# wonjune-kang/llm-speech-summarization

Measured on AMD Instinct MI355X. Metric: generated tokens/s of end-to-end generate_audio_response steps (encode + prefill + 256-token greedy decode), HuBERT-large -> Llama-3.2-3B; audio-sec/s reported beside it, encoder stage alone and in the pipeline, higher is better.
Workload: dtype bf16

## Files before the change

include/speechllm.h:

```cpp
#ifndef SPEECHLLM_H
#define SPEECHLLM_H

#include <stddef.h>
#include <stdint.h>

#ifdef __cplusplus
extern "C" {
#endif

typedef void* sl_stream;

enum sl_dtype { SL_F32 = 0, SL_BF16 = 1, SL_F16 = 2 };
enum sl_status {
  SL_OK = 0,
  SL_ERR_ARG = -1,
  SL_ERR_LAUNCH = -2,
  SL_ERR_UNSUPPORTED = -3
};
enum sl_act { SL_ACT_NONE = 0, SL_ACT_GELU = 1, SL_ACT_SILU_MUL = 2, SL_ACT_ROPE_KV = 3 };
enum sl_w_layout { SL_W_ROWMAJOR = 0, SL_W_PACKED = 1 };
#define SL_W_PACKED_E4M3 2
#define SL_W_PACKED_MXFP4 4

const char* sl_last_error(void);
// ... 22 lines not shown

size_t sl_w4_image_bytes(int32_t N, int32_t K);
int sl_pack_weight_mxfp4(const void* src, int64_t ld_src, void* dst, int32_t N, int32_t K, int32_t dtype, sl_stream stream);
int sl_pack_weight_mxfp4_host(const void* src, int64_t ld_src, void* dst, int32_t N, int32_t K, int32_t dtype);
int32_t sl_w4_max_rows(void);

size_t sl_mx_weight_image_bytes(int32_t N, int32_t K);
int sl_pack_weight_mx(const void* src, int64_t ld_src, void* dst, int32_t N, int32_t K, int32_t dtype, sl_stream stream);
int sl_pack_weight_mx_host(const void* src, int64_t ld_src, void* dst, int32_t N, int32_t K, int32_t dtype);
int sl_mxfp8_quantize_rows(const void* x, int64_t ldx, void* q, void* scales, int64_t M, int32_t K, int32_t dtype, sl_stream stream);
int sl_mxfp8_quantize_rows_host(const void* x, int64_t ldx, void* q, void* scales, int64_t M, int32_t K, int32_t dtype);
typedef struct {
  const void* Aq; int64_t lda; const void* a_scales;
  const void* W;
  void* C; int64_t ldc;
  const void* residual; int64_t ldr;
  int32_t M, N, K;
  int32_t dtype, act, out_f32;
} sl_gemm_mx_args;
int sl_gemm_mx(const sl_gemm_mx_args* a, sl_stream stream);

typedef struct {
  int32_t fuse_rms; float rms_eps;
  const float* rope_cos; const float* rope_sin;
  const int32_t* tok_pos; const int32_t* tok_seq;
  void* k_cache; void* v_cache;
  int32_t n_heads, n_kv_heads, max_ctx, reserved;
  void* split_ws; size_t split_ws_bytes;
  const float* rstd_in; float* rstd_out;
  void* norm_out; const void* norm_gain;
} sl_gemm_fused;
size_t sl_gemm_split_workspace_bytes(int32_t M, int32_t N, int32_t K, int32_t dtype);
int32_t sl_gemm_split_count(int32_t M, int32_t N, int32_t K, int32_t dtype);
int sl_gemm_fused_decode(const sl_gemm_args* a, const sl_gemm_fused* fx, sl_stream stream);

typedef struct {
  int32_t trans_a, trans_w, residual_f32, w_mod;
  void* aux_out;
  const int64_t* groups;
  int32_t groups_ext, reserved;
  float* amax_val; int32_t* amax_idx;
  const float* ln_mr; const float* ln_u; const float* ln_c; float* stats_out;
  void* sk_ws; size_t sk_ws_bytes;
  int32_t post_op, post_reserved;
  float drop_p; float post_reserved_f;
  uint64_t drop_seed;
  int64_t drop_ld;
  const void* post_in; int64_t post_ld;
  float* colsum_out;
  int32_t* deferred_splits;
} sl_gemm_ex_args;
enum { SL_POST_NONE = 0, SL_POST_DROPOUT = 1, SL_POST_GELU_BWD = 2, SL_POST_SILU_MUL_BWD = 3 };
int sl_gemm_ex(const sl_gemm_args* a, const sl_gemm_ex_args* ex, sl_stream stream);
size_t sl_gemm_streamk_workspace_bytes(void);
int32_t sl_gemm_ln_fold_ok(int32_t M, int32_t N, int32_t K, int32_t dtype);
int sl_layernorm_fold_build(const void* W, const void* gain, const void* beta, const void* bias, void* Wf, float* u, float* c, int32_t N,
                            int32_t K, int32_t dtype, sl_stream stream);
int sl_layernorm_stats_finalize(const float* stats, int32_t segs, int64_t rows, int32_t cols, float eps, float* mr, sl_stream stream);
int sl_layernorm_stats(const void* x, int64_t rows, int32_t cols, float eps, float* mr, int32_t dtype, sl_stream stream);

int sl_layernorm(const void* x, void* y, const void* gamma, const void* beta, int64_t rows, int32_t cols,
                 float eps, int32_t gelu, int32_t dtype, sl_stream stream);

int sl_rmsnorm(const void* x, void* y, const void* w, int64_t rows, int32_t cols, float eps, int32_t dtype,
               sl_stream stream);

// ... 516 lines not shown
```

llm-speech-summarization_amd/_lib.py:

```python
from __future__ import annotations

import ctypes as C
import os
from dataclasses import dataclass, field

import torch

_HERE = os.path.dirname(os.path.abspath(__file__))
LIB_PATH = (os.environ.get("SL_LIB_PATH") if os.environ.get("SL_DEV") == "1" else None) or os.path.join(_HERE, "libspeechllm.so")

SL_F32, SL_BF16, SL_F16 = 0, 1, 2
KV_MODEL_DTYPE, KV_FP8_E4M3 = 0, 1
ACT_NONE, ACT_GELU, ACT_SILU_MUL, ACT_ROPE_KV = 0, 1, 2, 3
POST_NONE, POST_DROPOUT, POST_GELU_BWD, POST_SILU_MUL_BWD = 0, 1, 2, 3
W_ROWMAJOR, W_PACKED, W_PACKED_E4M3 = 0, 1, 2
W_PACKED_MXFP4 = 4
WDEC_MODEL_DTYPE, WDEC_E4M3 = 0, 1
WDEC_MXFP4 = 4
WDEC_MX_LINEAR = 5
COMM_ID_BYTES = 128
MAX_DECODE_BATCH = 2048

c_i32, c_i64, c_f32, c_vp, c_sz = C.c_int32, C.c_int64, C.c_float, C.c_void_p, C.c_size_t

# ... 219 lines not shown
    "sl_tuning_reload": (c_i32, []),
    "sl_decode_graph_cache_clear": (c_i32, []),
    "sl_gemm": (c_i32, [C.POINTER(GemmArgs), c_vp]),
    "sl_gemm_streamk_workspace_bytes": (C.c_size_t, []),
    "sl_layernorm_fold_build": (c_i32, [c_vp, c_vp, c_vp, c_vp, c_vp, c_vp, c_vp, c_i32, c_i32, c_i32, c_vp]),
    "sl_weight_norm_bwd": (c_i32, [c_vp, c_vp, c_vp, c_vp, c_vp, c_vp, c_i32, c_i32, c_i32, c_vp]),
    "sl_weight_norm_bwd_workspace_bytes": (C.c_size_t, [c_i32]),
    "sl_comm_unique_id": (c_i32, [c_vp]),
    "sl_comm_init": (c_i32, [C.POINTER(c_vp), c_vp, c_i32, c_i32]),
    "sl_allreduce_sum": (c_i32, [c_vp, c_vp, c_i64, c_i32, c_vp]),
    "sl_comm_destroy": (c_i32, [c_vp]),
    "sl_comm_abort": (c_i32, [c_vp]),
    "sl_comm_rank": (c_i32, [c_vp]),
    "sl_comm_world": (c_i32, [c_vp]),
    "sl_pack_weight": (c_i32, [c_vp, c_i64, c_vp, c_i32, c_i32, c_i32, c_vp]),
    "sl_w8_image_bytes": (c_sz, [c_i32, c_i32]),
    "sl_pack_weight_e4m3": (c_i32, [c_vp, c_i64, c_vp, c_i32, c_i32, c_i32, c_vp]),
    "sl_pack_weight_e4m3_host": (c_i32, [c_vp, c_i64, c_vp, c_i32, c_i32, c_i32]),
    "sl_w8_max_rows": (c_i32, []),
    "sl_w4_image_bytes": (c_sz, [c_i32, c_i32]),
    "sl_pack_weight_mxfp4": (c_i32, [c_vp, c_i64, c_vp, c_i32, c_i32, c_i32, c_vp]),
    "sl_pack_weight_mxfp4_host": (c_i32, [c_vp, c_i64, c_vp, c_i32, c_i32, c_i32]),
    "sl_w4_max_rows": (c_i32, []),
    "sl_weight_format_info": (c_i32, [c_i32, C.POINTER(c_i32), C.POINTER(c_i32), C.POINTER(c_i32)]),
    "sl_mx_weight_image_bytes": (c_sz, [c_i32, c_i32]),
    "sl_pack_weight_mx": (c_i32, [c_vp, c_i64, c_vp, c_i32, c_i32, c_i32, c_vp]),
    "sl_pack_weight_mx_host": (c_i32, [c_vp, c_i64, c_vp, c_i32, c_i32, c_i32]),
    "sl_mxfp8_quantize_rows": (c_i32, [c_vp, c_i64, c_vp, c_vp, c_i64, c_i32, c_i32, c_vp]),
    "sl_mxfp8_quantize_rows_host": (c_i32, [c_vp, c_i64, c_vp, c_vp, c_i64, c_i32, c_i32]),
    "sl_gemm_mx": (c_i32, [C.POINTER(GemmMxArgs), c_vp]),
    "sl_gemm_fused_decode": (c_i32, [C.POINTER(GemmArgs), C.POINTER(GemmFused), c_vp]),
    "sl_gemm_split_workspace_bytes": (c_sz, [c_i32, c_i32, c_i32, c_i32]),
    "sl_gemm_split_count": (c_i32, [c_i32, c_i32, c_i32, c_i32]),
    "sl_attn_decode_workspace_bytes": (c_sz, [c_i32, c_i32, c_i32, c_i32]),
    "sl_attn_decode_split": (c_i32, [c_vp, c_i64, c_vp, c_vp, c_vp, c_vp, c_vp, c_i32, c_i32, c_i32, c_i32, c_i32, c_f32, c_i32, c_vp]),
    "sl_gemm_ex": (c_i32, [C.POINTER(GemmArgs), C.POINTER(GemmEx), c_vp]),
    "sl_gemm_ln_fold_ok": (c_i32, [c_i32, c_i32, c_i32, c_i32]),
    "sl_layernorm_stats_finalize": (c_i32, [c_vp, c_i32, c_i64, c_i32, c_f32, c_vp, c_vp]),
    "sl_layernorm_stats": (c_i32, [c_vp, c_i64, c_i32, c_f32, c_vp, c_i32, c_vp]),
    "sl_gelu_bwd": (c_i32, [c_vp, c_vp, c_vp, c_i64, c_i32, c_vp]),
    "sl_axpby": (c_i32, [c_vp, c_vp, c_f32, c_f32, c_i64, c_i32, c_vp]),
    "sl_adamw_blocks": (C.c_size_t, [c_i64]),
    "sl_adamw_step": (c_i32, [c_vp, c_vp, c_i32, c_i64, C.c_double, C.c_double, C.c_double, C.c_double, C.c_double, c_i64, c_vp]),
    "sl_attn_dropout_bwd": (c_i32, [c_vp, c_vp, c_vp, c_i64, c_i32, c_vp, c_i32, c_vp, c_i32, c_i32, c_i32, c_f32, C.c_uint64, c_i32, c_vp]),
    "sl_transpose_pad": (c_i32, [c_vp, c_i64, c_vp, c_i64, c_i32, c_i32, c_i32, c_i32, c_vp]),
    "sl_dropout": (c_i32, [c_vp, c_vp, c_vp, c_i64, c_f32, C.c_uint64, c_i32, c_vp]),
    "sl_silu_mul": (c_i32, [c_vp, c_vp, c_i64, c_i32, c_i32, c_vp]),
    "sl_silu_mul_bwd": (c_i32, [c_vp, c_vp, c_vp, c_i64, c_i32, c_i32, c_vp]),
    "sl_rope_inplace": (c_i32, [c_vp, c_vp, c_vp, c_vp, c_i64, c_i32, c_i32, c_i32, c_i32, c_i32, c_vp]),
    "sl_layernorm_bwd": (c_i32, [c_vp, c_vp, c_vp, c_vp, c_vp, c_vp, c_vp, c_i64, c_i32, c_f32, c_i32, c_i32, c_vp]),
    "sl_layernorm_bwd_ws_bytes": (c_sz, [c_i64, c_i32]),
    "sl_layernorm_bwd_ws": (c_i32, [c_vp, c_vp, c_vp, c_vp, c_vp, c_vp, c_vp, c_i64, c_i32, c_f32, c_i32, c_i32, c_vp, c_sz, c_vp]),
    "sl_rmsnorm_bwd": (c_i32, [c_vp, c_vp, c_vp, c_vp, c_i64, c_i32, c_f32, c_i32, c_vp]),
    "sl_colsum": (c_i32, [c_vp, c_i64, c_vp, c_i64, c_i32, c_i32, c_vp]),
    "sl_softmax_rows": (c_i32, [c_vp, c_vp, c_i64, c_i32, c_i32, c_i64, c_f32, c_i32, c_i32, c_vp]),
    "sl_softmax_bwd": (c_i32, [c_vp, c_vp, c_vp, c_i64, c_i32, c_i64, c_f32, c_i32, c_vp]),
    "sl_softmax_rows_var": (c_i32, [c_vp, c_vp, c_i64, c_i32, c_vp, c_i64, c_f32, c_i32, c_i32, c_vp]),
    "sl_softmax_bwd_var": (c_i32, [c_vp, c_vp, c_vp, c_i64, c_i32, c_vp, c_i64, c_f32, c_i32, c_vp]),
    "sl_ce_loss": (c_i32, [c_vp, c_vp, c_i64, c_i32, c_f32, c_vp, c_vp, c_i32, c_i32, c_vp]),
    "sl_soft_ce_loss": (c_i32, [c_vp, c_vp, c_i64, c_i32, c_f32, c_vp, c_vp, c_i32, c_i32, c_vp]),
    "sl_mse_loss": (c_i32, [c_vp, c_vp, c_i64, c_f32, c_vp, c_vp, c_i32, c_i32, c_vp]),
    "sl_kd_logit_losses": (c_i32, [c_vp, c_vp, c_vp, c_vp, c_vp, c_i64, c_i32, c_vp, c_i32, c_vp, c_i32, c_vp]),
    "sl_kd_mse_rows": (c_i32, [c_vp, c_vp, c_vp, c_vp, c_i64, c_i32, c_vp, c_i32, c_i32, c_vp, c_i32, c_vp]),
    "sl_avgpool_bwd": (c_i32, [c_vp, c_vp, c_i64, c_i32, c_i32, c_i32, c_i64, c_i32, c_vp]),
    "sl_col2im": (c_i32, [c_vp, c_vp, c_i64, c_i64, c_i32, c_i32, c_i32, c_i32, c_vp]),
    "sl_col2im_batch": (c_i32, [c_vp, c_vp, c_vp, c_i32, c_i64, c_i32, c_i32, c_i32, c_i32, c_vp]),
# ... 248 lines not shown
```

llm-speech-summarization_amd/csrc/api.hip:

```cpp
#include <stdarg.h>
#include <stdlib.h>

#include <atomic>
#include <mutex>

#include "common.h"

static thread_local char g_err[512] = "";

void sl_set_error(const char* fmt, ...) {
  va_list ap;
  va_start(ap, fmt);
  vsnprintf(g_err, sizeof(g_err), fmt, ap);
  va_end(ap);
}

extern "C" const char* sl_last_error(void) { return g_err; }

extern "C" int sl_version(void) { return SL_ABI_VERSION; }

extern "C" int sl_kv_quantize_e4m3_host(const float* x, uint8_t* out, int64_t n) {
  SL_CHECK_ARG(x != nullptr && out != nullptr && n >= 0, "sl_kv_quantize_e4m3_host: bad arguments");
  for (int64_t i = 0; i < n; ++i) out[i] = (uint8_t)sl_q8_e4m3(x[i]);
  return 0;
// ... 46 lines not shown
  e.t256_min_k = env_int("SL_T256_MIN_K", 1024);
  e.t256_phased = env_int("SL_T256_PHASED", 1);
  e.t256_by_rounds_pad = env_int("SL_T256_BY_ROUNDS_PAD", 1);
  e.decode_tiled = env_int("SL_DECODE_TILED", 1);
  e.stream_k = env_int("SL_STREAM_K", 1);
  e.split_k = env_int("SL_SPLIT_K", 1);
  e.wgrad_tr = env_int("SL_WGRAD_TR", 1);
  e.tt_max_splits = env_int("SL_TT_MAX_SPLITS", 8);
  e.lnbwd_nw = env_int("SL_LNBWD_NW", 16);
  e.skinny_alt = env_int("SL_SKINNY_ALT", 0);
  e.prefill_share_prefix = env_int("SL_PREFILL_SHARE_PREFIX", 1);
  e.prefill_prune_last = env_int("SL_PREFILL_PRUNE_LAST", 1);
  e.gemm_ko = env_int("SL_GEMM_KO", 0);
  { const char* sp = getenv("SL_GEMM_STAMP_PTR"); e.gemm_stamp_ptr = (sp && sp[0]) ? strtoull(sp, nullptr, 16) : 0ull; }
  const char* g = getenv("SL_DISABLE_GLDS");
  e.disable_glds = (g && g[0] == '1') ? 1 : ((g && g[0] == '2') ? 2 : 0);
  e.direct_epilogue = env_int("SL_DIRECT_EPILOGUE", 0);
  e.gemm_gm = env_int("SL_GEMM_GM", 8);
  e.attn_full_min = env_int("SL_ATTN_FULL_MIN", 32);
  e.attn_force_split = getenv("SL_ATTN_FORCE_SPLIT") != nullptr;
  { const int ks = env_int("SL_ATTN_DECODE_KS", 128); e.attn_decode_ks = (ks == 64 || ks == 65) ? ks : 128; }
  e.attn_split_merge = env_int("SL_ATTN_SPLIT_MERGE", -1);
  e.attn_generic = env_int("SL_ATTN_GENERIC", 0);
  e.attn_qt = env_int("SL_ATTN_QT", 0);
  e.norm_single_row = env_int("SL_NORM_SINGLE_ROW", 0);
  e.no_ln_fold = env_int("SL_NO_LN_FOLD", 0);
  e.no_swap_epilogue = env_int("SL_NO_SWAP_EPILOGUE", 0);
  e.gemm_log = env_int("SL_GEMM_LOG", 0);
  e.no_wgrad_stream = env_int("SL_NO_WGRAD_STREAM", 0);
  e.stream_splits = e.stream_nwv = e.stream_mt = 0;
  e.stream_nl = env_int("SL_STREAM_NL", 0);
  e.stream_wide = env_int("SL_STREAM_WIDE", 1);
  e.stream_wsplits = env_int("SL_STREAM_WSPLITS", 0);
  e.stream_fixup = env_int("SL_STREAM_FIXUP", 0);
  const char* sc = getenv("SL_STREAM_CFG");
  if (sc && sc[0]) {
    int sp = 0, nwv = 0, mt = 0;
    const int n = sscanf(sc, "%d,%d,%d", &sp, &nwv, &mt);
    if (n >= 2) {
      if (sp >= 1 && sp <= 64) e.stream_splits = sp;
      if (nwv == 2 || nwv == 4) e.stream_nwv = nwv;
    }
    if (n == 3 && (mt == 8 || mt == 16)) e.stream_mt = mt;
  }
  return &e;
}

const SlEnv& sl_env() {
  const SlEnv* e = g_env.load(std::memory_order_acquire);
  if (!e) {
    std::lock_guard<std::mutex> lk(g_env_mu);
    e = g_env.load(std::memory_order_relaxed);
    if (!e) {
      e = env_load();
      g_env.store(e, std::memory_order_release);
    }
  }
  return *e;
}

static thread_local int g_family_rows = 0;
int sl_family_rows(int rows) { return g_family_rows > rows ? g_family_rows : rows; }
int sl_family_pin(int rows) {
  const int prev = g_family_rows;
  g_family_rows = rows > 0 ? rows : 0;
  return prev;
}
// ... 7 lines not shown
```

llm-speech-summarization_amd/csrc/gemm.hip:

```cpp
#include <stdlib.h>

#include "common.h"
#include "gemm_internal.h"
#include "wformat.h"

#include "gemm_epilogue.h"

template <typename T, int ACT>
__global__ __launch_bounds__(256, 2) void gemm_tiled_kernel(GemmP p) {
  constexpr int VEC = Vec16<T>::VEC;
  constexpr int BK = TROWB / (int)sizeof(T);
  __shared__ __attribute__((aligned(16))) unsigned char smem[2][2][TBM * TROWB];

  const int tid = threadIdx.x, lane = tid & 63, wave = tid >> 6;
  const int wm = wave >> 1, wn = wave & 1;
  const int r = lane & 15, q = lane >> 4;

  int bm, bn;
  tile_patch_coords(xcd_remap(blockIdx.x, p.tiles_m * p.tiles_n), p.tiles_m, p.tiles_n, 8, bm, bn);
  const int z = blockIdx.y;

  int64_t a_off; int wz;
  if (!resolve_group(p, z, bm, a_off, wz)) return;
  const T* A = (const T*)p.A + a_off;
// ... 1155 lines not shown
  const size_t sk_ws_bytes = ex ? ex->sk_ws_bytes : 0;
  SL_CHECK_ARG(!sk_ws || ((uintptr_t)sk_ws & 15) == 0, "sl_gemm_ex: sk_ws must be 16-byte aligned");
  if (a->dtype == SL_F32) return gemm_typed<float>(a, p, sx, st, sk_ws, sk_ws_bytes, e);
  if (a->dtype == SL_F16) return gemm_typed<f16_t>(a, p, sx, st, sk_ws, sk_ws_bytes, e);
  return gemm_typed<bf16_t>(a, p, sx, st, sk_ws, sk_ws_bytes, e);
}

int sl_gemm_impl(const sl_gemm_args* a, const sl_gemm_fused* fx, const sl_gemm_ex_args* ex, hipStream_t st) { return gemm_impl(a, fx, ex, st, nullptr); }

int sl_gemm_top1_lse_impl(const sl_gemm_args* a, const sl_gemm_ex_args* ex, float* amax_sum, hipStream_t st) {
  SL_CHECK_ARG(ex != nullptr && amax_sum != nullptr, "sl_gemm_top1_lse: null ex args or amax_sum");
  return gemm_impl(a, nullptr, ex, st, amax_sum);
}

extern "C" int sl_gemm_top1_lse(const sl_gemm_args* a, const sl_gemm_ex_args* ex, float* amax_sum, sl_stream stream) {
  return sl_gemm_top1_lse_impl(a, ex, amax_sum, (hipStream_t)stream);
}

int sl_gemm_top1_lse_tgt_impl(const sl_gemm_args* a, const sl_gemm_ex_args* ex, float* amax_sum, const int32_t* tgt_col, float* tgt_val, hipStream_t st) {
  SL_CHECK_ARG(ex != nullptr && amax_sum != nullptr, "sl_gemm_top1_lse_tgt: null ex args or amax_sum");
  return gemm_impl(a, nullptr, ex, st, amax_sum, tgt_col, tgt_val);
}

extern "C" int sl_gemm_top1_lse_tgt(const sl_gemm_args* a, const sl_gemm_ex_args* ex, float* amax_sum, const int32_t* tgt_col, float* tgt_val, sl_stream stream) {
  return sl_gemm_top1_lse_tgt_impl(a, ex, amax_sum, tgt_col, tgt_val, (hipStream_t)stream);
}

extern "C" int32_t sl_gemm_split_count(int32_t M, int32_t N, int32_t K, int32_t dtype) {
  M = sl_family_rows(M);
  if (M <= sl_env().stream_min_m || M <= 0 || N <= 0 || K <= 0 || K % (dtype == SL_F32 ? 32 : 64) != 0) return 1;
  return sl_gemm_stream_splits(M, N, K, dtype);
}

extern "C" size_t sl_gemm_split_workspace_bytes(int32_t M, int32_t N, int32_t K, int32_t dtype) {
  if (sl_family_rows(M) <= sl_env().stream_min_m || M <= 0 || N <= 0 || K <= 0) return 0;
  return sl_gemm_stream_ws_bytes(M, N, K, dtype);
}

extern "C" int32_t sl_gemm_ln_fold_ok(int32_t M, int32_t N, int32_t K, int32_t dtype) { return sl_gemm_rows_epilogue_ok(M, N, K, dtype) ? 1 : 0; }

extern "C" int sl_gemm(const sl_gemm_args* a, sl_stream stream) { return sl_gemm_impl(a, nullptr, nullptr, (hipStream_t)stream); }

extern "C" int sl_gemm_ex(const sl_gemm_args* a, const sl_gemm_ex_args* ex, sl_stream stream) {
  SL_CHECK_ARG(ex != nullptr, "sl_gemm_ex: null ex args");
  return sl_gemm_impl(a, nullptr, ex, (hipStream_t)stream);
}

extern "C" int sl_gemm_fused_decode(const sl_gemm_args* a, const sl_gemm_fused* fx, sl_stream stream) {
  SL_CHECK_ARG(fx != nullptr, "sl_gemm_fused_decode: null fused args");
  return sl_gemm_impl(a, fx, nullptr, (hipStream_t)stream);
}
```

llm-speech-summarization_amd/csrc/gemm_internal.h:

```cpp
#pragma once
#include "common.h"

struct GemmP {
  const void* A; int64_t lda, sA;
  const void* W; int64_t ldw, sW;
  void* C; int64_t ldc, sC;
  const void* bias; int64_t sBias;
  const void* res; int64_t ldr, sR;
  int M, N, K, out_f32;
  int tiles_m, tiles_n;
  int ta, tw;
  void* aux;
  int res_f32;
  const int64_t* grp;
  int w_mod;
  int64_t cx, rx, wx;
  int grp_ext;
  int grp_kslab;
  int gm;
  int direct_epi;
  const float* ln_mr;
  const float* ln_u;
  const float* ln_c;
  float* stats_out;
// ... 109 lines not shown
int sl_gemm128_ring_launch(const GemmP& p, int stages, dim3 grid, hipStream_t st);
enum : int { SL_TT_TWO_STAGE = 0, SL_TT_RING = 1, SL_TT_BATCHED = 2 };
int sl_gemm_tt_kernel_launch(const GemmP& p, int form, dim3 grid, int slabs_per_run, hipStream_t st);

bool sl_gemm_post_ok(int64_t M, int N, int K, int dtype);
bool sl_gemm_rows_epilogue_ok(int M, int N, int K, int dtype);

struct SkinnyX {
  const float* cos; const float* sin;
  const int32_t* pos; const int32_t* seq;
  void* kc; void* vc;
  int nh, nkv, max_ctx, fuse_rms;
  float eps;
  int kv8;
  const float* rstd_in;
  float* rstd_out;
  void* norm_out;
  const void* norm_gain;
};
constexpr int SL_ACT_ROPE_KV8 = 64 + SL_ACT_ROPE_KV;
constexpr bool sl_act_is_rope_kv(int act) { return act == SL_ACT_ROPE_KV || act == SL_ACT_ROPE_KV8; }
template <typename T>
__device__ __forceinline__ void kv_store(void* cache, int64_t at, float v, int kv8) {
  const T t = from_f32<T>(v);
  if constexpr (sizeof(T) == 2) {
    if (kv8) { ((uint8_t*)cache)[at] = (uint8_t)sl_q8_e4m3(to_f32(t)); return; }
  }
  ((T*)cache)[at] = t;
}

int sl_gemm_stream_launch(GemmP& p, const SkinnyX& sx, int dtype, int act, void* split_ws, size_t split_ws_bytes, hipStream_t st);
size_t sl_gemm_stream_ws_bytes(int M, int N, int K, int dtype);
int sl_gemm_stream_splits(int M, int N, int K, int dtype);
```

llm-speech-summarization_amd/csrc/gemm_stream.hip:

```cpp
#include <type_traits>
#include <stdlib.h>

#include <atomic>

#include "gemm_internal.h"

struct StreamX {
  float* part;
  float* part_ss;
  int splits, sps;
  int np;
  int* cnt;
  float* ss_part;
};

__device__ __forceinline__ void st_sc1_16(float* ptr, const f32x4& v) {
  asm volatile("global_store_dwordx4 %0, %1, off sc1" ::"v"(ptr), "v"(v) : "memory");
}
__device__ __forceinline__ void ld_sc1_16(f32x4& v, const float* ptr) {
  asm volatile("global_load_dwordx4 %0, %1, off sc1" : "=v"(v) : "v"(ptr) : "memory");
}
__device__ __forceinline__ void vm_drain16(f32x4 (&v)[16]) {
  asm volatile("s_waitcnt vmcnt(0)"
               : "+v"(v[0]), "+v"(v[1]), "+v"(v[2]), "+v"(v[3]), "+v"(v[4]), "+v"(v[5]), "+v"(v[6]), "+v"(v[7]), "+v"(v[8]), "+v"(v[9]), "+v"(v[10]),
                 "+v"(v[11]), "+v"(v[12]), "+v"(v[13]), "+v"(v[14]), "+v"(v[15])
               :
               : "memory");
}

template <typename T, int ACT>
__device__ __forceinline__ void stream_epilogue4(const GemmP& p, const SkinnyX& sx, int m, int gf, int n4, const float (&a)[4], const float (&b)[4]) {
  const T* bias = (const T*)p.bias;
  if constexpr (ACT == SL_ACT_SILU_MUL) {
    const int ocol = (gf >> 1) * 16 + n4;
    if (ocol >= (p.N >> 1)) return;
#pragma unroll
    for (int i = 0; i < 4; ++i) {
      float g = a[i], u = b[i];
      if (bias) { g += to_f32(bias[gf * 16 + n4 + i]); u += to_f32(bias[(gf + 1) * 16 + n4 + i]); }
      store_out<T>(p, p.C, p.res, m, ocol + i, silu(g) * u);
    }
  } else if constexpr (ACT == SL_ACT_ROPE_KV) {
    if (gf * 16 >= p.N) return;
    const int hh = gf >> 3, j = (gf & 7) >> 1;
    const int pos = sx.pos[m];
    if (hh < sx.nh + sx.nkv) {
// ... 257 lines not shown
    for (int d = 0; d < D - 1; ++d)
      if (n_full + d < n_it) stage(d, n_full + d);
    if constexpr (FUSE) {
#pragma unroll
      for (int j = 0; j < NSS; ++j) {
        const int t = j * NWV + wn;
        if (t < MT && (r >> 2) == q) ssl[t * 16 + r] = ssacc[j][r & 3];
      }
    }
  }
  __syncthreads();
  if (wave >= NWV) return;

  float ssum[MT];
#pragma unroll
  for (int t = 0; t < MT; ++t) {
    ssum[t] = 0.f;
    if (fuse) ssum[t] = ssl[t * 16 + r];
  }
  stream_finish<T, MT, ACT, RF>(p, sx, s, acc, ssum, fuse, m0, sp, fi0, nfrag, nb == 0 && wn == 0, q, r);
}

template <typename T, int ACT>
__global__ __launch_bounds__(768) void gemm_stream_wide_kernel(GemmP p, SkinnyX sx, StreamX s) {
  constexpr int VEC = Vec16<T>::VEC;
  constexpr int KSTEP = MMA<T>::KSTEP;
  constexpr int CW = 8;
  constexpr int MTW = 4, RFW = 4;
  constexpr int BM = 256, BF = 8;
  constexpr int SLAB_X = BM * TROWB, SLAB_W = BF * 2 * 1024, SLOT = SLAB_X + SLAB_W;
  constexpr int NSLOT = 3;
  constexpr int NDMA = 12;
  extern __shared__ __attribute__((aligned(16))) unsigned char smem[];
  __shared__ int fx_last[2];
  __shared__ float fx_ss[4][2][64];

  const int tid = threadIdx.x, lane = tid & 63;
  const int wave = __builtin_amdgcn_readfirstlane(tid >> 6);
  const int r = lane & 15, q = lane >> 4;
  const int mblocks = (p.M + BM - 1) / BM;
  const int nfrag = (p.N + 15) >> 4;
  const int xj = blockIdx.x >> 3, nb = (xj / mblocks) * 8 + (blockIdx.x & 7);
  if (nb * BF >= nfrag) return;
  const int mblock = xj % mblocks;
  const int m0 = mblock * BM;
  const int sp = blockIdx.z;
  const int nks = p.K / KSTEP;
  const int g_lo = sp * s.sps;
  const int g_hi = min(nks >> 1, g_lo + s.sps);
  const int n_it = g_hi - g_lo;
  const int g_last = g_hi - 1;
  const int wm = (wave >> 1) & 3, wn = wave & 1;
  const int mw = m0 + wm * 64, fi0 = nb * BF + wn * RFW;

  f32x4 acc[RFW][MTW];
  float ssum[MTW];
#pragma unroll
  for (int t = 0; t < MTW; ++t) {
    ssum[t] = 0.f;
#pragma unroll
    for (int f = 0; f < RFW; ++f) acc[f][t] = f32x4{0.f, 0.f, 0.f, 0.f};
  }

  if (wave >= CW) {
    const int lw = wave - CW;
    const T* A = (const T*)p.A;
    const T* W = (const T*)p.W;
    const int ch = (lane & 7) ^ ((lane >> 3) & 7);
// ... 56 lines not shown
      }
    };
    __builtin_amdgcn_s_barrier();
    rd(0, 0, 0);
    for (int it = 0; it < n_it; ++it) {
      __builtin_amdgcn_sched_barrier(0);
      rd(it, 1, 1);
      mma(0);
      __builtin_amdgcn_sched_barrier(0);
      asm volatile("s_waitcnt lgkmcnt(0)" ::: "memory");
      __builtin_amdgcn_s_barrier();
      rd(it + 1, 0, 0);
      mma(1);
      __builtin_amdgcn_sched_barrier(0);
    }
    stream_finish<T, MTW, ACT, RFW>(p, sx, s, acc, ssum, false, mw, sp, fi0, nfrag, false, q, r);
  }
  if (!(s.splits > 1 && s.cnt)) return;

  const bool cw = wave < CW;
  const int tile = nb * mblocks + mblock;
  asm volatile("s_waitcnt vmcnt(0)" ::: "memory");
  __builtin_amdgcn_s_barrier();
  if (tid == 0) {
    const int old = atomicAdd(&s.cnt[tile], 1);
    fx_last[0] = old == s.splits - 1;
    if (old == s.splits - 1) s.cnt[tile] = 0;
  }
  __builtin_amdgcn_s_barrier();
  if (!fx_last[0]) return;
  bool rowstat = false;
  if constexpr (ACT == SL_ACT_NONE) rowstat = sx.rstd_out != nullptr;
  if (cw) {
#pragma unroll
    for (int t = 0; t < MTW; ++t)
#pragma unroll
      for (int f = 0; f < RFW; ++f) acc[f][t] = f32x4{0.f, 0.f, 0.f, 0.f};
    for (int sp2 = 0; sp2 < s.splits; ++sp2) {
      f32x4 v[MTW * RFW];
#pragma unroll
      for (int t = 0; t < MTW; ++t) {
        int m = mw + t * 16 + r; m = m < p.M ? m : p.M - 1;
#pragma unroll
        for (int f = 0; f < RFW; ++f) {
          const int fi = fi0 + f < nfrag ? fi0 + f : nfrag - 1;
          ld_sc1_16(v[t * RFW + f], s.part + ((int64_t)sp2 * p.M + m) * s.np + fi * 16 + 4 * q);
        }
      }
      vm_drain16(v);
#pragma unroll
      for (int t = 0; t < MTW; ++t)
#pragma unroll
        for (int f = 0; f < RFW; ++f) acc[f][t] += v[t * RFW + f];
    }
    if (!rowstat) {
      StreamX s1 = s;
      s1.splits = 1;
      stream_finish<T, MTW, ACT, RFW>(p, sx, s1, acc, ssum, false, mw, sp, fi0, nfrag, false, q, r);
    }
  }
  if (!rowstat) return;
  if constexpr (ACT == SL_ACT_NONE) {
    if (cw) {
      const T* bias = (const T*)p.bias;
#pragma unroll
      for (int t = 0; t < MTW; ++t) {
        const int m = mw + t * 16 + r;
        float sq = 0.f;
        if (m < p.M) {
#pragma unroll
          for (int f = 0; f < RFW; ++f) {
#pragma unroll
            for (int i = 0; i < 4; ++i) {
              const int col = (fi0 + f) * 16 + 4 * q + i;
              if (col >= p.N) continue;
              float v = acc[f][t][i];
              if (bias) v += to_f32(bias[col]);
              if (p.res) v += p.res_f32 ? ((const float*)p.res)[(int64_t)m * p.ldr + col] : to_f32(((const T*)p.res)[(int64_t)m * p.ldr + col]);
              if (p.out_f32) {
                ((float*)p.C)[(int64_t)m * p.ldc + col] = v;
              } else {
                const T o = from_f32<T>(v);
                ((T*)p.C)[(int64_t)m * p.ldc + col] = o;
                v = to_f32(o);
              }
              sq = fmaf(v, v, sq);
            }
          }
        }
        sq += __shfl_xor(sq, 16);
        sq += __shfl_xor(sq, 32);
        if (q == 0) fx_ss[wm][wn][t * 16 + r] = sq;
      }
    }
    const int nbv = (nfrag + BF - 1) / BF;
    __builtin_amdgcn_s_barrier();
    if (tid < 256) {
      const int m = m0 + tid;
      if (m < p.M)
        __hip_atomic_store(&s.ss_part[(int64_t)nb * p.M + m], fx_ss[tid >> 6][0][tid & 63] + fx_ss[tid >> 6][1][tid & 63], __ATOMIC_RELAXED,
                           __HIP_MEMORY_SCOPE_AGENT);
    }
    asm volatile("s_waitcnt vmcnt(0)" ::: "memory");
    __builtin_amdgcn_s_barrier();
    if (tid == 0) {
      const int old = atomicAdd(&s.cnt[1024 + mblock], 1);
      fx_last[1] = old == nbv - 1;
      if (old == nbv - 1) s.cnt[1024 + mblock] = 0;
    }
    __builtin_amdgcn_s_barrier();
    if (!fx_last[1]) return;
    if (tid < 256) {
      const int m = m0 + tid;
      if (m < p.M) {
        float t = 0.f;
        for (int j = 0; j < nbv; ++j) t += __hip_atomic_load(&s.ss_part[(int64_t)j * p.M + m], __ATOMIC_RELAXED, __HIP_MEMORY_SCOPE_AGENT);
        sx.rstd_out[m] = rsqrtf(t / (float)p.N + sx.eps);
      }
    }
  }
}

template <int UN, int NCH, bool PAIRS>
__device__ __forceinline__ void reduce_add_splits(const float* rec, int64_t split_stride, int sp0, const uint32_t (&voff)[NCH], f32x4 (&a4)[NCH],
                                                  f32x4 (&b4)[NCH]) {
  f32x4 va[NCH][UN], vb[NCH][UN];
#pragma unroll
  for (int u = 0; u < UN; ++u) {
    const float* row = rec + (int64_t)(sp0 + u) * split_stride;
#pragma unroll
    for (int j = 0; j < NCH; ++j) {
      va[j][u] = *(const f32x4*)(row + voff[j]);
      if constexpr (PAIRS) vb[j][u] = *(const f32x4*)(row + voff[j] + 16);
    }
  }
#pragma unroll
  for (int u = 0; u < UN; ++u)
#pragma unroll
    for (int j = 0; j < NCH; ++j) {
      a4[j] += va[j][u];
      if constexpr (PAIRS) b4[j] += vb[j][u];
    }
}
template <int UNMAX, int NCH, bool PAIRS>
__device__ __forceinline__ void reduce_sum_splits(const float* rec, int64_t split_stride, int splits, const uint32_t (&voff)[NCH], f32x4 (&a4)[NCH],
                                                  f32x4 (&b4)[NCH]) {
  int sp0 = 0;
  for (; sp0 + UNMAX <= splits; sp0 += UNMAX) reduce_add_splits<UNMAX, NCH, PAIRS>(rec, split_stride, sp0, voff, a4, b4);
  if constexpr (UNMAX > 4) {
// ... 240 lines not shown
  const int mblocks = (M + c.mt * 16 - 1) / (c.mt * 16);
  c.nwv = ((nfrag + 7) / 8 * mblocks >= 512 || M > 128) && c.mt <= 8 ? 4 : 2;
  if (nwv_env && c.mt <= 8) c.nwv = nwv_env;
  const int base = mblocks * ((nfrag + c.nwv * 2 - 1) / (c.nwv * 2));
  int splits = 1;
  if (have_ws) {
    splits = 208 / base;
    const int max_splits = nst / 4 > 0 ? nst / 4 : 1;
    if (splits > max_splits) splits = max_splits;
    if (splits > 16) splits = 16;
    if (splits < 1) splits = 1;
  }
  if (sp_env && (have_ws || sp_env == 1)) splits = sp_env < nst ? sp_env : nst;
  c.splits = splits;
  c.wide = 0; c.wsplits = 1;
  if (sl_is16(dtype) && M > 384 && sl_env().stream_wide != 0) {
    const int wbase = ((M + 255) / 256) * ((nfrag + 7) / 8);
    if (wbase >= 128 || sl_env().stream_wide == 2) {
      c.wide = 1;
    }
    if (wbase < 128 && have_ws) {
      int ws_ = 240 / wbase;
      const int max_ws = nst / 6 > 0 ? nst / 6 : 1;
      if (ws_ > max_ws) ws_ = max_ws;
      if (ws_ > 8) ws_ = 8;
      if (sl_env().stream_wsplits) ws_ = sl_env().stream_wsplits < nst ? sl_env().stream_wsplits : nst;
      if (ws_ > 1) { c.wide = 1; c.wsplits = ws_; }
    }
  }
  return c;
}

static size_t stream_ws_header(int M) { return 8192 + (((size_t)32 * M * sizeof(float) + 255) & ~(size_t)255); }

int sl_gemm_stream_splits(int M, int N, int K, int dtype) {
  const StreamCfg c = stream_cfg(sl_family_rows(M), N, K, dtype == SL_F32 ? 16 : 32, true, dtype);
  return c.wide ? c.wsplits : c.splits;
}

size_t sl_gemm_stream_ws_bytes(int M, int N, int K, int dtype) {
  const size_t np = (size_t)((N + 15) / 16) * 16;
  const StreamCfg c = stream_cfg(sl_family_rows(M), N, K, dtype == SL_F32 ? 16 : 32, true, dtype);
  const int most = c.wide && c.wsplits > c.splits ? c.wsplits : c.splits;
  size_t splits = most > 1 ? (size_t)most : 0;
  return stream_ws_header(M) + splits * ((size_t)M * np + (size_t)M) * sizeof(float) + 256;
}

template <typename T, int ACT>
static int launch_stream_reduce(GemmP& p, const SkinnyX& sx, const StreamX& s, hipStream_t st) {
  if (s.splits <= 1) return 0;
  constexpr bool PAIRS = (ACT == SL_ACT_SILU_MUL || sl_act_is_rope_kv(ACT));
  const int nfrag = (p.N + 15) / 16;
  const int64_t nunits = PAIRS ? (nfrag + 1) / 2 : nfrag;
  const int64_t threads = (int64_t)p.M * nunits * 4;
  if constexpr (ACT == SL_ACT_NONE) {
    if (sx.rstd_out) {
      const uintptr_t al = sizeof(T) == 2 ? 7 : 15;
      const bool fast = !p.bias && p.res && !p.res_f32 && !p.out_f32 && !sx.fuse_rms && !sx.rstd_in && !(p.N & 3) && !(p.ldc & 3) && !(p.ldr & 3) &&
                        !((uintptr_t)p.C & al) && !((uintptr_t)p.res & al) && (!sx.norm_out || (!((uintptr_t)sx.norm_out & al) && !((uintptr_t)sx.norm_gain & al)));
      const int nch = (nfrag * 4 + 255) / 256;
#define SL_ROWSTAT_LAUNCH(NCH_)                                                                                                              \
  if (fast) hipLaunchKernelGGL((gemm_stream_reduce_rowstat_kernel<T, NCH_, true>), dim3(p.M), dim3(256), 0, st, p, sx, s);                   \
  else hipLaunchKernelGGL((gemm_stream_reduce_rowstat_kernel<T, NCH_, false>), dim3(p.M), dim3(256), 0, st, p, sx, s)
      if (nch <= 1) { SL_ROWSTAT_LAUNCH(1); }
      else if (nch == 2) { SL_ROWSTAT_LAUNCH(2); }
      else if (nch == 3) { SL_ROWSTAT_LAUNCH(3); }
      else { SL_ROWSTAT_LAUNCH(4); }
#undef SL_ROWSTAT_LAUNCH
      SL_CHECK_LAUNCH("gemm_stream_reduce(rowstat)");
      return 0;
    }
  }
  hipLaunchKernelGGL((gemm_stream_reduce_kernel<T, ACT>), dim3((unsigned)((threads + 255) / 256)), dim3(256), 0, st, p, sx, s);
  SL_CHECK_LAUNCH("gemm_stream_reduce");
  return 0;
}

template <typename T, int MT, int ACT, int RF, int NWV, int D, int NL>
// ... 27 lines not shown
    }
  }
}

template <typename T, int ACT>
static int launch_stream(GemmP& p, const SkinnyX& sx, const StreamX& s, const StreamCfg& c, hipStream_t st) {
  switch (c.mt) {
    case 2: return launch_stream_mt<T, 2, ACT>(p, sx, s, c, st);
    case 4: return launch_stream_mt<T, 4, ACT>(p, sx, s, c, st);
    case 8: return launch_stream_mt<T, 8, ACT>(p, sx, s, c, st);
    default: return launch_stream_mt<T, 16, ACT>(p, sx, s, c, st);
  }
}

template <typename T>
static int stream_typed(GemmP& p, const SkinnyX& sx, int act, const StreamX& s, const StreamCfg& c, hipStream_t st) {
  switch (act) {
    case SL_ACT_NONE: return launch_stream<T, SL_ACT_NONE>(p, sx, s, c, st);
    case SL_ACT_SILU_MUL: return launch_stream<T, SL_ACT_SILU_MUL>(p, sx, s, c, st);
    case SL_ACT_ROPE_KV:
      if constexpr (sizeof(T) == 2) { if (sx.kv8) return launch_stream<T, SL_ACT_ROPE_KV8>(p, sx, s, c, st); }
      return launch_stream<T, SL_ACT_ROPE_KV>(p, sx, s, c, st);
  }
  sl_set_error("sl_gemm: packed weights are not built with act %d for M > 16 streaming", act);
  return SL_ERR_UNSUPPORTED;
}

static bool stream_wide_ok(const SkinnyX& sx, int act, const StreamCfg& c, bool have_ws) {
  if (!c.wide || (sx.fuse_rms != 0 && sx.rstd_in == nullptr)) return false;
  if (act != SL_ACT_NONE && act != SL_ACT_SILU_MUL && act != SL_ACT_ROPE_KV) return false;
  return c.wsplits == 1 || have_ws;
}

template <typename T, int ACT>
static int launch_stream_wide_act(GemmP& p, const SkinnyX& sx, const StreamX& s, hipStream_t st) {
  const int nfrag = (p.N + 15) / 16, mblocks = (p.M + 255) / 256, nblocks = (nfrag + 7) / 8;
  constexpr int LDS_BYTES = 3 * (256 * TROWB + 8 * 2 * 1024);
  dim3 grid((nblocks + 7) / 8 * 8 * mblocks, 1, s.splits);
  static std::atomic<uint64_t> attr_set{0};
  int devid = 0;
  SL_HIP(hipGetDevice(&devid));
  if (devid < 0 || devid >= 64 || !((attr_set.load(std::memory_order_relaxed) >> devid) & 1)) {
    SL_HIP(hipFuncSetAttribute((const void*)gemm_stream_wide_kernel<T, ACT>, hipFuncAttributeMaxDynamicSharedMemorySize, LDS_BYTES));
    if (devid >= 0 && devid < 64) attr_set.fetch_or(1ull << devid, std::memory_order_relaxed);
  }
  hipLaunchKernelGGL((gemm_stream_wide_kernel<T, ACT>), grid, dim3(768), LDS_BYTES, st, p, sx, s);
  SL_CHECK_LAUNCH("gemm_stream_wide");
  if (s.cnt) return 0;
  return launch_stream_reduce<T, ACT>(p, sx, s, st);
}

template <typename T>
static int launch_stream_wide(GemmP& p, const SkinnyX& sx, int act, const StreamX& s, hipStream_t st) {
  switch (act) {
    case SL_ACT_SILU_MUL: return launch_stream_wide_act<T, SL_ACT_SILU_MUL>(p, sx, s, st);
    case SL_ACT_ROPE_KV:
      if constexpr (sizeof(T) == 2) { if (sx.kv8) return launch_stream_wide_act<T, SL_ACT_ROPE_KV8>(p, sx, s, st); }
      return launch_stream_wide_act<T, SL_ACT_ROPE_KV>(p, sx, s, st);
    default: return launch_stream_wide_act<T, SL_ACT_NONE>(p, sx, s, st);
  }
}

int sl_gemm_stream_launch(GemmP& p, const SkinnyX& sx, int dtype, int act, void* split_ws, size_t split_ws_bytes, hipStream_t st) {
  const int kstep = dtype == SL_F32 ? 16 : 32;
  SL_CHECK_ARG(p.K % (2 * kstep) == 0, "sl_gemm: streaming path needs K %% %d == 0 (K=%d)", 2 * kstep, p.K);
  StreamCfg c = stream_cfg(sl_family_rows(p.M), p.N, p.K, kstep, split_ws != nullptr, dtype);
  StreamX s;
  const bool wide = stream_wide_ok(sx, act, c, split_ws != nullptr);
  if (wide) c.splits = c.wsplits;

  s.np = (p.N + 15) / 16 * 16;
  const size_t per_split = ((size_t)p.M * s.np + (size_t)p.M) * sizeof(float);
  const size_t hdr = stream_ws_header(p.M);
  split_ws_bytes = (split_ws && split_ws_bytes > hdr) ? split_ws_bytes - hdr : 0;
  if (c.splits > 1 && (size_t)c.splits * per_split > split_ws_bytes) c.splits = (int)(split_ws_bytes / per_split);
  if (c.splits < 1) c.splits = 1;
  const int nst = p.K / (2 * kstep);
  s.sps = (nst + c.splits - 1) / c.splits;
  s.splits = (nst + s.sps - 1) / s.sps;
  c.splits = s.splits;
  SL_CHECK_ARG(sx.norm_out == nullptr || sx.rstd_out != nullptr, "sl_gemm: norm_out comes from the pass that forms rstd_out (pass both)");
  if (sx.rstd_out) {
    SL_CHECK_ARG(act == SL_ACT_NONE && (p.N + 15) / 16 * 4 <= 1024 && s.splits > 1,
                 "sl_gemm: rstd_out needs the plain epilogue, N <= 4096 and a K-split (splits=%d; see sl_gemm_split_count)", s.splits);
  }
  s.part = split_ws ? (float*)((unsigned char*)split_ws + hdr) : nullptr;
  s.part_ss = s.part ? s.part + (size_t)s.splits * p.M * s.np : nullptr;
  s.cnt = nullptr; s.ss_part = nullptr;
  if (wide && s.splits > 1 && sl_env().stream_fixup != 0 && sx.norm_out == nullptr) {
    const int nbv = ((p.N + 15) / 16 + 7) / 8, mbl = (p.M + 255) / 256;
    if (nbv * mbl <= 1024 && mbl <= 64 && (sx.rstd_out == nullptr || nbv <= 32)) {
      s.cnt = (int*)split_ws;
      s.ss_part = (float*)((unsigned char*)split_ws + 8192);
    }
  }
  if (dtype == SL_F32) return stream_typed<float>(p, sx, act, s, c, st);
  if (dtype == SL_F16) {
    if (wide) return launch_stream_wide<f16_t>(p, sx, act, s, st);
    return stream_typed<f16_t>(p, sx, act, s, c, st);
  }
  if (wide) return launch_stream_wide<bf16_t>(p, sx, act, s, st);
  return stream_typed<bf16_t>(p, sx, act, s, c, st);
}
```

Measured before the change: 68600.

## Enable in-launch split-K fixup by default for two-split wide stream GEMMs

Changes the default of the stream fixup mode to an automatic setting that closes the K-split reduction inside the GEMM launch when there are exactly two splits and the family row count exceeds 896. This removes the separate reduce kernel launch. It also reworks the rowstat (rstd) path: per-block squared sums are staged in LDS, and neighbouring N-blocks are paired through a global pieces buffer and a pair counter, which halves the number of partial sums the last block must gather. The split-2 path reduces the peer split into the existing accumulators instead of re-summing every split. In exchange the workspace grows and more inter-block atomic handshakes are needed. A query API reports whether a given shape will close its split in-launch.

```diff
diff --git a/include/speechllm.h b/include/speechllm.h
--- a/include/speechllm.h
+++ b/include/speechllm.h
@@ -78,6 +78,7 @@
 } sl_gemm_fused;
 size_t sl_gemm_split_workspace_bytes(int32_t M, int32_t N, int32_t K, int32_t dtype);
 int32_t sl_gemm_split_count(int32_t M, int32_t N, int32_t K, int32_t dtype);
+int32_t sl_gemm_split_closes_in_launch(int32_t M, int32_t family_rows, int32_t N, int32_t K, int32_t dtype, int32_t norm_out);
 int sl_gemm_fused_decode(const sl_gemm_args* a, const sl_gemm_fused* fx, sl_stream stream);
 
 typedef struct {
diff --git a/llm-speech-summarization_amd/_lib.py b/llm-speech-summarization_amd/_lib.py
--- a/llm-speech-summarization_amd/_lib.py
+++ b/llm-speech-summarization_amd/_lib.py
@@ -275,6 +275,7 @@
     "sl_gemm_fused_decode": (c_i32, [C.POINTER(GemmArgs), C.POINTER(GemmFused), c_vp]),
     "sl_gemm_split_workspace_bytes": (c_sz, [c_i32, c_i32, c_i32, c_i32]),
     "sl_gemm_split_count": (c_i32, [c_i32, c_i32, c_i32, c_i32]),
+    "sl_gemm_split_closes_in_launch": (c_i32, [c_i32, c_i32, c_i32, c_i32, c_i32, c_i32]),
     "sl_attn_decode_workspace_bytes": (c_sz, [c_i32, c_i32, c_i32, c_i32]),
     "sl_attn_decode_split": (c_i32, [c_vp, c_i64, c_vp, c_vp, c_vp, c_vp, c_vp, c_i32, c_i32, c_i32, c_i32, c_i32, c_f32, c_i32, c_vp]),
     "sl_gemm_ex": (c_i32, [C.POINTER(GemmArgs), C.POINTER(GemmEx), c_vp]),
diff --git a/llm-speech-summarization_amd/csrc/api.hip b/llm-speech-summarization_amd/csrc/api.hip
--- a/llm-speech-summarization_amd/csrc/api.hip
+++ b/llm-speech-summarization_amd/csrc/api.hip
@@ -102,7 +102,7 @@
   e.stream_nl = env_int("SL_STREAM_NL", 0);
   e.stream_wide = env_int("SL_STREAM_WIDE", 1);
   e.stream_wsplits = env_int("SL_STREAM_WSPLITS", 0);
-  e.stream_fixup = env_int("SL_STREAM_FIXUP", 0);
+  e.stream_fixup = env_int("SL_STREAM_FIXUP", -1);
   const char* sc = getenv("SL_STREAM_CFG");
   if (sc && sc[0]) {
     int sp = 0, nwv = 0, mt = 0;
diff --git a/llm-speech-summarization_amd/csrc/gemm.hip b/llm-speech-summarization_amd/csrc/gemm.hip
--- a/llm-speech-summarization_amd/csrc/gemm.hip
+++ b/llm-speech-summarization_amd/csrc/gemm.hip
@@ -1211,6 +1211,12 @@
   return sl_gemm_stream_splits(M, N, K, dtype);
 }
 
+extern "C" int32_t sl_gemm_split_closes_in_launch(int32_t M, int32_t family_rows, int32_t N, int32_t K, int32_t dtype, int32_t norm_out) {
+  SlFamilyPin pin(family_rows > 0 ? family_rows : sl_family_rows(0));
+  if (sl_gemm_split_count(M, N, K, dtype) <= 1) return 0;
+  return sl_gemm_stream_closes_in_launch(M, N, K, dtype, norm_out != 0);
+}
+
 extern "C" size_t sl_gemm_split_workspace_bytes(int32_t M, int32_t N, int32_t K, int32_t dtype) {
   if (sl_family_rows(M) <= sl_env().stream_min_m || M <= 0 || N <= 0 || K <= 0) return 0;
   return sl_gemm_stream_ws_bytes(M, N, K, dtype);
diff --git a/llm-speech-summarization_amd/csrc/gemm_internal.h b/llm-speech-summarization_amd/csrc/gemm_internal.h
--- a/llm-speech-summarization_amd/csrc/gemm_internal.h
+++ b/llm-speech-summarization_amd/csrc/gemm_internal.h
@@ -165,3 +165,4 @@
 int sl_gemm_stream_launch(GemmP& p, const SkinnyX& sx, int dtype, int act, void* split_ws, size_t split_ws_bytes, hipStream_t st);
 size_t sl_gemm_stream_ws_bytes(int M, int N, int K, int dtype);
 int sl_gemm_stream_splits(int M, int N, int K, int dtype);
+int sl_gemm_stream_closes_in_launch(int M, int N, int K, int dtype, bool norm_out);
diff --git a/llm-speech-summarization_amd/csrc/gemm_stream.hip b/llm-speech-summarization_amd/csrc/gemm_stream.hip
--- a/llm-speech-summarization_amd/csrc/gemm_stream.hip
+++ b/llm-speech-summarization_amd/csrc/gemm_stream.hip
@@ -12,6 +12,7 @@
   int np;
   int* cnt;
   float* ss_part;
+  float* pieces;
 };
 
 __device__ __forceinline__ void st_sc1_16(float* ptr, const f32x4& v) {
@@ -335,8 +336,7 @@
   constexpr int NSLOT = 3;
   constexpr int NDMA = 12;
   extern __shared__ __attribute__((aligned(16))) unsigned char smem[];
-  __shared__ int fx_last[2];
-  __shared__ float fx_ss[4][2][64];
+  __shared__ int fx_last[3];
 
   const int tid = threadIdx.x, lane = tid & 63;
   const int wave = __builtin_amdgcn_readfirstlane(tid >> 6);
@@ -459,11 +459,14 @@
   bool rowstat = false;
   if constexpr (ACT == SL_ACT_NONE) rowstat = sx.rstd_out != nullptr;
   if (cw) {
-#pragma unroll
-    for (int t = 0; t < MTW; ++t)
-#pragma unroll
-      for (int f = 0; f < RFW; ++f) acc[f][t] = f32x4{0.f, 0.f, 0.f, 0.f};
-    for (int sp2 = 0; sp2 < s.splits; ++sp2) {
+    const int sp_lo = s.splits == 2 ? (sp ^ 1) : 0, sp_hi = s.splits == 2 ? (sp ^ 1) + 1 : s.splits;
+    if (s.splits != 2) {
+#pragma unroll
+      for (int t = 0; t < MTW; ++t)
+#pragma unroll
+        for (int f = 0; f < RFW; ++f) acc[f][t] = f32x4{0.f, 0.f, 0.f, 0.f};
+    }
+    for (int sp2 = sp_lo; sp2 < sp_hi; ++sp2) {
       f32x4 v[MTW * RFW];
 #pragma unroll
       for (int t = 0; t < MTW; ++t) {
@@ -488,15 +491,17 @@
   }
   if (!rowstat) return;
   if constexpr (ACT == SL_ACT_NONE) {
+    constexpr int PCW = 36;
+    float* pc = (float*)smem;
     if (cw) {
       const T* bias = (const T*)p.bias;
 #pragma unroll
       for (int t = 0; t < MTW; ++t) {
         const int m = mw + t * 16 + r;
-        float sq = 0.f;
-        if (m < p.M) {
-#pragma unroll
-          for (int f = 0; f < RFW; ++f) {
+#pragma unroll
+        for (int f = 0; f < RFW; ++f) {
+          float sq = 0.f;
+          if (m < p.M) {
 #pragma unroll
             for (int i = 0; i < 4; ++i) {
               const int col = (fi0 + f) * 16 + 4 * q + i;
@@ -514,34 +519,72 @@
               sq = fmaf(v, v, sq);
             }
           }
+          pc[(wm * 64 + t * 16 + r) * PCW + wn * 16 + f * 4 + q] = sq;
         }
-        sq += __shfl_xor(sq, 16);
-        sq += __shfl_xor(sq, 32);
-        if (q == 0) fx_ss[wm][wn][t * 16 + r] = sq;
-      }
-    }
-    const int nbv = (nfrag + BF - 1) / BF;
-    __builtin_amdgcn_s_barrier();
+      }
+    }
+    const int nbv = (nfrag + BF - 1) / BF, ngr = (nbv + 1) >> 1;
+    const int nbp = nb ^ 1;
+    __syncthreads();
+    if (nbp < nbv) {
+#pragma unroll
+      for (int i = 0; i < 3; ++i) {
+        const int j = tid + 768 * i, row = j >> 3, c4 = j & 7;
+        if (j < 2048 && m0 + row < p.M)
+          st_sc1_16(s.pieces + ((int64_t)nb * p.M + m0 + row) * 32 + c4 * 4, *(const f32x4*)(pc + row * PCW + c4 * 4));
+      }
+      asm volatile("s_waitcnt vmcnt(0)" ::: "memory");
+      __builtin_amdgcn_s_barrier();
+      if (tid == 0) {
+        int* pair = &s.cnt[1088 + (nb >> 1) * mblocks + mblock];
+        const int old = atomicAdd(pair, 1);
+        fx_last[1] = old == 1;
+        if (old == 1) *pair = 0;
+      }
+      __builtin_amdgcn_s_barrier();
+      if (!fx_last[1]) return;
+      f32x4 pv[3];
+#pragma unroll
+      for (int i = 0; i < 3; ++i) {
+        const int j = min(tid + 768 * i, 2047), c4 = j & 7;
+        const int m = min(m0 + (j >> 3), p.M - 1);
+        ld_sc1_16(pv[i], s.pieces + ((int64_t)nbp * p.M + m) * 32 + c4 * 4);
+      }
+      asm volatile("s_waitcnt vmcnt(0)" : "+v"(pv[0]), "+v"(pv[1]), "+v"(pv[2]) : : "memory");
+#pragma unroll
+      for (int i = 0; i < 3; ++i) {
+        const int j = tid + 768 * i, row = j >> 3, c4 = j & 7;
+        if (j < 2048 && m0 + row < p.M) *(f32x4*)(pc + row * PCW + c4 * 4) += pv[i];
+      }
+      __syncthreads();
+    }
     if (tid < 256) {
       const int m = m0 + tid;
-      if (m < p.M)
-        __hip_atomic_store(&s.ss_part[(int64_t)nb * p.M + m], fx_ss[tid >> 6][0][tid & 63] + fx_ss[tid >> 6][1][tid & 63], __ATOMIC_RELAXED,
-                           __HIP_MEMORY_SCOPE_AGENT);
+      if (m < p.M) {
+        float w[16];
+#pragma unroll
+        for (int l = 0; l < 16; ++l) w[l] = pc[tid * PCW + l] + pc[tid * PCW + l + 16];
+#pragma unroll
+        for (int o = 8; o > 0; o >>= 1)
+#pragma unroll
+          for (int l = 0; l < o; ++l) w[l] = w[l] + w[l + o];
+        __hip_atomic_store(&s.ss_part[(int64_t)(nb >> 1) * p.M + m], w[0], __ATOMIC_RELAXED, __HIP_MEMORY_SCOPE_AGENT);
+      }
     }
     asm volatile("s_waitcnt vmcnt(0)" ::: "memory");
     __builtin_amdgcn_s_barrier();
     if (tid == 0) {
       const int old = atomicAdd(&s.cnt[1024 + mblock], 1);
-      fx_last[1] = old == nbv - 1;
-      if (old == nbv - 1) s.cnt[1024 + mblock] = 0;
+      fx_last[2] = old == ngr - 1;
+      if (old == ngr - 1) s.cnt[1024 + mblock] = 0;
     }
     __builtin_amdgcn_s_barrier();
-    if (!fx_last[1]) return;
+    if (!fx_last[2]) return;
     if (tid < 256) {
       const int m = m0 + tid;
       if (m < p.M) {
         float t = 0.f;
-        for (int j = 0; j < nbv; ++j) t += __hip_atomic_load(&s.ss_part[(int64_t)j * p.M + m], __ATOMIC_RELAXED, __HIP_MEMORY_SCOPE_AGENT);
+        for (int j = 0; j < ngr; ++j) t += __hip_atomic_load(&s.ss_part[(int64_t)j * p.M + m], __ATOMIC_RELAXED, __HIP_MEMORY_SCOPE_AGENT);
         sx.rstd_out[m] = rsqrtf(t / (float)p.N + sx.eps);
       }
     }
@@ -848,6 +891,7 @@
 }
 
 static size_t stream_ws_header(int M) { return 8192 + (((size_t)32 * M * sizeof(float) + 255) & ~(size_t)255); }
+static size_t stream_piece_bytes(int M, int N) { return (size_t)(((N + 15) / 16 + 7) / 8) * M * 32 * sizeof(float); }
 
 int sl_gemm_stream_splits(int M, int N, int K, int dtype) {
   const StreamCfg c = stream_cfg(sl_family_rows(M), N, K, dtype == SL_F32 ? 16 : 32, true, dtype);
@@ -859,7 +903,8 @@
   const StreamCfg c = stream_cfg(sl_family_rows(M), N, K, dtype == SL_F32 ? 16 : 32, true, dtype);
   const int most = c.wide && c.wsplits > c.splits ? c.wsplits : c.splits;
   size_t splits = most > 1 ? (size_t)most : 0;
-  return stream_ws_header(M) + splits * ((size_t)M * np + (size_t)M) * sizeof(float) + 256;
+  const size_t pieces = c.wide && c.wsplits > 1 ? 256 + stream_piece_bytes(M, N) : 0;
+  return stream_ws_header(M) + splits * ((size_t)M * np + (size_t)M) * sizeof(float) + 256 + pieces;
 }
 
 template <typename T, int ACT>
@@ -953,6 +998,19 @@
   return c.wsplits == 1 || have_ws;
 }
 
+static bool stream_close_in_launch(int family_rows, bool wide, int splits, bool norm_out) {
+  if (!wide || splits < 2 || norm_out) return false;
+  const int mode = sl_env().stream_fixup;
+  return mode < 0 ? (splits == 2 && family_rows > 896) : mode != 0;
+}
+
+int sl_gemm_stream_closes_in_launch(int M, int N, int K, int dtype, bool norm_out) {
+  const int kstep = dtype == SL_F32 ? 16 : 32;
+  const StreamCfg c = stream_cfg(sl_family_rows(M), N, K, kstep, true, dtype);
+  const int nst = K / (2 * kstep), sps = (nst + c.wsplits - 1) / c.wsplits;
+  return c.wide && stream_close_in_launch(sl_family_rows(M), true, (nst + sps - 1) / sps, norm_out) ? 1 : 0;
+}
+
 template <typename T, int ACT>
 static int launch_stream_wide_act(GemmP& p, const SkinnyX& sx, const StreamX& s, hipStream_t st) {
   const int nfrag = (p.N + 15) / 16, mblocks = (p.M + 255) / 256, nblocks = (nfrag + 7) / 8;
@@ -1007,12 +1065,15 @@
   }
   s.part = split_ws ? (float*)((unsigned char*)split_ws + hdr) : nullptr;
   s.part_ss = s.part ? s.part + (size_t)s.splits * p.M * s.np : nullptr;
-  s.cnt = nullptr; s.ss_part = nullptr;
-  if (wide && s.splits > 1 && sl_env().stream_fixup != 0 && sx.norm_out == nullptr) {
+  s.cnt = nullptr; s.ss_part = nullptr; s.pieces = nullptr;
+  if (stream_close_in_launch(sl_family_rows(p.M), wide, s.splits, sx.norm_out != nullptr)) {
     const int nbv = ((p.N + 15) / 16 + 7) / 8, mbl = (p.M + 255) / 256;
-    if (nbv * mbl <= 1024 && mbl <= 64 && (sx.rstd_out == nullptr || nbv <= 32)) {
+    const size_t pieces_at = ((size_t)s.splits * per_split + 255) & ~(size_t)255;
+    const bool pieces_fit = pieces_at + stream_piece_bytes(p.M, p.N) <= split_ws_bytes;
+    if (nbv * mbl <= 1024 && mbl <= 64 && (sx.rstd_out == nullptr || (nbv <= 32 && pieces_fit))) {
       s.cnt = (int*)split_ws;
       s.ss_part = (float*)((unsigned char*)split_ws + 8192);
+      s.pieces = (float*)((unsigned char*)s.part + pieces_at);
     }
   }
   if (dtype == SL_F32) return stream_typed<float>(p, sx, act, s, c, st);
```

Result: slower. 66760 (-2.7%).
